# youngsm/chroma-lite

Hardware: AMD Instinct MI355X
Metric: propagated photons/sec, 29k-PMT detector, 10M isotropic photons, 1/2/4/8 GPUs (higher is better)
Workload: dtype f32

## Files before the change

chroma-lite_amd/chroma/gpu/_native.py:

```python
import ctypes
import os

_LIBDIR = os.path.join(os.path.dirname(os.path.dirname(os.path.abspath(__file__))), '_lib')
DEVICE_PROFILE = os.environ.get('CHROMA_DEVICE_PROFILE', '').strip().lower() in ('1', 'true', 'yes', 'on')
_LIBPATH = os.path.join(_LIBDIR, 'libchroma_amd_prof.so' if DEVICE_PROFILE else 'libchroma_amd.so')
_LIBPATH = os.environ.get('CHROMA_AMD_LIB', _LIBPATH)

c_u32 = ctypes.c_uint32
c_i32 = ctypes.c_int32
c_u64 = ctypes.c_uint64
c_f32 = ctypes.c_float
c_vp = ctypes.c_void_p
P_f32 = ctypes.POINTER(ctypes.c_float)
P_u32 = ctypes.POINTER(ctypes.c_uint32)


class MaterialDesc(ctypes.Structure):
    _fields_ = [('num_comp', c_u32), ('refractive_index', c_vp), ('absorption_length', c_vp),
                ('scattering_length', c_vp), ('comp_reemission_prob', c_vp),
                ('comp_reemission_wvl_cdf', c_vp), ('comp_reemission_time_cdf', c_vp),
                ('comp_absorption_length', c_vp)]


class SurfaceDesc(ctypes.Structure):
# ... 46 lines not shown
                ('tail_long_ticks', c_u64), ('tail_long_walk_ticks', c_u64), ('tail_long_walk_iterations', c_u64),
                ('host_syncs', c_u32), ('tail_long_paired_steps', c_u32), ('trace_launch_rays', c_u32 * 32)]


class KernelAttr(ctypes.Structure):
    _fields_ = [('private_bytes', c_u64), ('lds_bytes', c_u64), ('vgprs', ctypes.c_int32),
                ('max_threads', ctypes.c_int32), ('name', ctypes.c_char * 96)]


_SIGNATURES = {
    'chr_geometry_create': (c_i32, [ctypes.POINTER(GeometryDesc), ctypes.POINTER(c_vp)]),
    'chr_geometry_destroy': (c_i32, [c_vp]),
    'chr_geometry_device_bytes': (c_i32, [c_vp, ctypes.POINTER(c_u64)]),
    'chr_walk_lone_timing': (c_i32, [c_vp, c_vp, c_u32, c_u32, c_u32, c_i32, c_vp, c_vp]),
    'chr_geometry_phys_words': (c_i32, [c_vp, ctypes.POINTER(ctypes.c_uint32), ctypes.POINTER(ctypes.c_uint32)]),
    'chr_init_rng': (c_i32, [c_vp, c_u32, c_u64, c_u64, c_vp]),
    'chr_rng_download': (c_i32, [c_vp, c_u32, c_vp, c_vp]),
    'chr_propagate_scratch_words': (c_u64, [c_u32]),
    'chr_propagate_chunk': (c_i32, [c_vp, ctypes.POINTER(PhotonsDesc), c_vp, c_u32, c_i32, c_i32, c_vp, c_vp,
                                    c_i32, c_i32, c_i32, c_vp, c_vp]),
    'chr_propagate': (c_i32, [c_vp, ctypes.POINTER(PhotonsDesc), c_u32, c_u32, c_u32, c_vp, c_u32, c_i32, c_i32,
                              c_i32, c_i32, c_i32, ctypes.POINTER(PropagateStats), c_vp]),
    'chr_propagate_batches': (c_i32, [c_vp, ctypes.POINTER(PhotonsDesc), c_vp, c_vp, c_vp, c_u32, c_vp, c_u32, c_i32,
                                      c_i32, c_i32, c_i32, c_i32, ctypes.POINTER(PropagateStats), c_vp]),
    'chr_photon_hits': (c_i32, [ctypes.POINTER(PhotonsDesc), c_i32, c_i32, c_u32, c_vp, c_vp,
                                ctypes.POINTER(PhotonsDesc), c_vp, ctypes.POINTER(c_u32), c_vp]),
    'chr_select_photons': (c_i32, [ctypes.POINTER(PhotonsDesc), c_i32, c_i32, c_u32, ctypes.POINTER(PhotonsDesc),
                                   ctypes.POINTER(c_u32), c_vp]),
    'chr_copy_photon_queue': (c_i32, [ctypes.POINTER(PhotonsDesc), c_i32, c_i32, c_vp, ctypes.POINTER(PhotonsDesc),
                                      c_vp]),
# ... 92 lines not shown
    if rc != 0:
        msg = lib().chr_last_error().decode(errors='replace')
        raise NativeError('%s failed (status %d): %s' % (what, rc, msg))
    return rc


call_hook = None


def call(name, *args):
    if call_hook is not None:
        return call_hook(name, lambda: check(getattr(lib(), name)(*args), name))
    return check(getattr(lib(), name)(*args), name)


def kernel_info():
    out = []
    for which in range(4):
        a = KernelAttr()
        call('chr_kernel_info', which, ctypes.byref(a))
        out.append(dict(name=a.name.decode(), private_bytes=int(a.private_bytes), lds_bytes=int(a.lds_bytes),
                        vgprs=int(a.vgprs), max_threads=int(a.max_threads)))
    return out


def set_host_threads(n):
    call('chr_set_host_threads', int(n))


def host_threads():
    return int(lib().chr_get_host_threads())
```

chroma-lite_amd/chroma/gpu/geometry.py:

```python
import ctypes
import time

import numpy as np

from chroma.gpu import _native, wide_bvh
from chroma.gpu import gpuarray as ga
from chroma.gpu.packing import PackedGeometry
from chroma.gpu.tools import format_size
from chroma.log import logger


class GPUGeometry(object):
    def __init__(self, geometry, wavelengths=None, times=None, print_usage=False, min_free_gpu_mem=300e6):
        t0 = time.time()
        if getattr(geometry, 'bvh', None) is None:
            from chroma.loader import load_bvh
            geometry.bvh = load_bvh(geometry)
        self.packed = PackedGeometry(geometry, wavelengths=wavelengths, times=times)
        t1 = time.time()
        wide, source = wide_bvh.obtain(geometry.bvh, self.packed)
        t2 = time.time()
        handle = ctypes.c_void_p()
        try:
            _native.call('chr_geometry_create_wide', ctypes.byref(self.packed.desc()), ctypes.byref(wide.desc()),
# ... 44 lines not shown
        if getattr(self, '_triangles', None) is None:
            from chroma.gpu.tools import to_uint3
            self._triangles = ga.to_gpu(to_uint3(self.packed.triangles))
        return self._triangles

    def device_bytes(self):
        b = ctypes.c_uint64()
        _native.call('chr_geometry_device_bytes', self._handle, ctypes.byref(b))
        return b.value

    def phys_words(self):
        hot, total = ctypes.c_uint32(), ctypes.c_uint32()
        _native.call('chr_geometry_phys_words', self._handle, ctypes.byref(hot), ctypes.byref(total))
        return hot.value, total.value

    def device_usage_str(self):
        return 'device usage: geometry %s (%d triangles, %d BVH nodes)' % (
            format_size(self.device_bytes()), len(self.packed.triangles), len(self.packed.nodes))

    def print_device_usage(self):
        print(self.device_usage_str())

    def __del__(self):
        h = getattr(self, '_handle', None)
        if h is not None and h.value:
            try:
                _native.lib().chr_geometry_destroy(h)
            except Exception:
                pass
            self._handle = ctypes.c_void_p()
# ... 1 lines not shown
```

chroma-lite_amd/csrc/device_geometry.h:

```cpp
#pragma once
#include <vector>

#include <cstdint>

#include "../../include/chroma_amd.h"

namespace chr {

constexpr uint32_t TIME_INDEX_BUCKETS = 4096;

struct DevMaterial {
    uint32_t num_comp;
    uint32_t refractive_index, absorption_length, scattering_length;
    uint32_t comp_reemission_prob, comp_reemission_wvl_cdf, comp_absorption_length;
    uint32_t comp_reemission_time_cdf;
    uint32_t comp_time_index;
};

struct DevSurface {
    uint32_t present, model, transmissive;
    float thickness;
    uint32_t detect, absorb, reemit, reflect_diffuse, reflect_specular, eta, k, reemission_cdf;
    uint32_t dichroic_nangles, dichroic_angles, dichroic_reflect, dichroic_transmit;
    uint32_t angular_nangles, angular_angles, angular_transmit, angular_reflect_specular,
// ... 11 lines not shown
    const uint4 *wnodes;
    const float4 *wtri;
    uint32_t nwnodes, nwtri;
    uint32_t wstride;
    float ox, oy, oz, scale;
    float wbound;
    uint32_t nnodes, ntriangles, nwireplanes;
    uint32_t wl_n;
    float wl_start, wl_step;
    uint32_t t_n;
    float t_start, t_step;
    const uint32_t *phys;
    uint32_t phys_words, mat_off, surf_off;
    uint32_t phys_hot_words;
    const float *tables_g;
};

}

struct chr_geometry {
    chr::DevGeom dev;
    void *d_dev;
    int device;
    uint64_t bytes;
    void *allocs[16];
    int nallocs;
    std::vector<uint4> *h_ref_nodes;
    bool ref_tri_pending;
};
namespace chr {
// ... 5 lines not shown
```

chroma-lite_amd/csrc/geometry.cpp:

```cpp
#include <hip/hip_runtime_api.h>

#include <algorithm>
#include <cmath>
#include <cstdlib>
#include <cstring>
#include <mutex>
#include <new>
#include <string>
#include <unordered_map>
#include <vector>

#include "../../include/chroma_amd.h"
#include "common.h"
#include "slab_plane.h"
#include "wide_bvh.h"
#include "device_geometry.h"

namespace chr {
std::string &last_error() {
    static thread_local std::string msg;
    return msg;
}
}

// ... 100 lines not shown
    const int rc = run();
    if (prev != g->device) (void)hipSetDevice(prev);
    return rc;
}

extern "C" int chr_geometry_device_bytes(const chr_geometry *g, uint64_t *bytes) {
    if (!g || !bytes) return chr::fail(CHR_ERR_INVALID, "chr_geometry_device_bytes: null argument");
    *bytes = g->bytes;
    return CHR_OK;
}

extern "C" int chr_geometry_phys_words(const chr_geometry *g, uint32_t *hot_words, uint32_t *total_words) {
    if (!g || !hot_words || !total_words) return chr::fail(CHR_ERR_INVALID, "chr_geometry_phys_words: null argument");
    *hot_words = g->dev.phys_hot_words;
    *total_words = g->dev.phys_words;
    return CHR_OK;
}

struct Stager {
    static constexpr size_t CHUNK = 64u << 20;
    hipStream_t stream = nullptr;
    void *buf[2] = {nullptr, nullptr};
    hipEvent_t ev[2] = {nullptr, nullptr};
    bool used[2] = {false, false};
    std::vector<uint8_t> pageable;
    int init() {
        if (hipStreamCreateWithFlags(&stream, hipStreamNonBlocking) != hipSuccess) stream = nullptr;
        for (int k = 0; k < 2 && stream; ++k) {
            if (hipHostMalloc(&buf[k], CHUNK, hipHostMallocDefault) != hipSuccess ||
                hipEventCreateWithFlags(&ev[k], hipEventDisableTiming) != hipSuccess) {
// ... 175 lines not shown

        if ((rc = dev_upload(g, d->h_material_codes, (size_t)d->ntriangles * 4, &p))) throw rc;
        dg.material_codes = (const uint32_t *)p;

        Blob blob, comp;
        const uint32_t W1 = d->wavelength_n + 1, T1 = d->time_n + 1;
        std::vector<chr::DevMaterial> mats(d->nmaterials);
        for (uint32_t i = 0; i < d->nmaterials; ++i) {
            const chr_material_desc &m = d->materials[i];
            chr::DevMaterial &o = mats[i];
            if (!m.refractive_index || !m.absorption_length || !m.scattering_length) {
                rc = chr::fail(CHR_ERR_INVALID, "material %u: missing table", i);
                throw rc;
            }
            o.num_comp = m.num_comp;
            o.refractive_index = blob.add(m.refractive_index, W1);
            o.absorption_length = blob.add(m.absorption_length, W1);
            o.scattering_length = blob.add(m.scattering_length, W1);
            const size_t nc = m.num_comp;
            o.comp_reemission_prob = blob.add(m.comp_reemission_prob, nc * W1);
            o.comp_reemission_wvl_cdf = blob.add(m.comp_reemission_wvl_cdf, nc * W1);
            o.comp_absorption_length = blob.add(m.comp_absorption_length, nc * W1);
            o.comp_reemission_time_cdf = comp.add(m.comp_reemission_time_cdf, nc * T1);
            o.comp_time_index = ~0u;
            std::vector<uint32_t> idx;
            if (nc && chr::time_cdf_index(m.comp_reemission_time_cdf, m.num_comp, d->time_n, T1, idx))
                o.comp_time_index = comp.add(idx.data(), idx.size());
        }
        std::vector<chr::DevSurface> surfs(d->nsurfaces > 0 ? d->nsurfaces : 1);
        std::memset(surfs.data(), 0, surfs.size() * sizeof(chr::DevSurface));
        for (uint32_t i = 0; i < d->nsurfaces; ++i) {
            const chr_surface_desc &s = d->surfaces[i];
            chr::DevSurface &o = surfs[i];
            o.present = s.present ? 1u : 0u;
            if (!s.present) continue;
            o.model = s.model; o.transmissive = s.transmissive; o.thickness = s.thickness;
            o.detect = blob.add(s.detect, W1);
            o.absorb = blob.add(s.absorb, W1);
            o.reemit = blob.add(s.reemit, W1);
            o.reflect_diffuse = blob.add(s.reflect_diffuse, W1);
            o.reflect_specular = blob.add(s.reflect_specular, W1);
            o.eta = blob.add(s.eta, W1);
            o.k = blob.add(s.k, W1);
            o.reemission_cdf = blob.add(s.reemission_cdf, W1);
            if (s.model == CHR_SURFACE_DICHROIC && s.dichroic_nangles == 0) {
                rc = chr::fail(CHR_ERR_INVALID, "surface %u: dichroic model without DichroicProps", i);
                throw rc;
            }
            if (s.model == CHR_SURFACE_ANGULAR && s.angular_nangles == 0) {
                rc = chr::fail(CHR_ERR_INVALID, "surface %u: angular model without AngularProps", i);
                throw rc;
// ... 32 lines not shown
            phys.resize(phys.size() + comp.data.size());
            std::memcpy(phys.data() + hot, comp.data.data(), comp.data.size() * 4);
            phys.resize((phys.size() + 3) & ~(size_t)3, 0u);
            if ((rc = dev_upload(g, phys.data(), phys.size() * 4, &p))) throw rc;
            dg.phys = (const uint32_t *)p;
            dg.phys_words = (uint32_t)phys.size();
            dg.phys_hot_words = hot;
            dg.mat_off = mat_off;
            dg.surf_off = surf_off;
            dg.tables = (const float *)p;
            dg.tables_g = (const float *)p;
            dg.materials = (const chr::DevMaterial *)(dg.phys + mat_off);
            dg.surfaces = (const chr::DevSurface *)(dg.phys + surf_off);
        }
        if (d->nwireplanes) {
            if ((rc = dev_upload(g, d->wireplanes, (size_t)d->nwireplanes * sizeof(chr_wireplane_desc), &p))) throw rc;
            dg.wireplanes = (const chr_wireplane_desc *)p;
        }
        if ((rc = dev_upload(g, &dg, sizeof(dg), &p))) throw rc;
        g->d_dev = p;
    } catch (int code) {
        chr_geometry_destroy(g);
        return code;
    } catch (const std::bad_alloc &) {
        chr_geometry_destroy(g);
        return chr::fail(CHR_ERR_NOMEM, "chr_geometry_create: host allocation failed");
    }
    *out = g;
    return CHR_OK;
}
// ... 10 lines not shown
```

chroma-lite_amd/csrc/propagate.hip:

```cpp
#include <hip/hip_runtime.h>
#include <rocprim/device/device_radix_sort.hpp>

#include <algorithm>
#include <cstdint>
#include <cstdio>
#include <cstdlib>
#include <cstring>
#include <functional>
#include <type_traits>
#include <vector>

#include "../../include/chroma_amd.h"
#include "../../include/chroma_fmath.h"
#include "../../include/chroma_rng.h"
#include "common.h"
#include "device_geometry.h"
#include "device_math.h"
#include "sampling.h"
#include "slab_plane.h"
#include "wide_bvh.h"

namespace chr {

constexpr int BLOCK = 256;
constexpr int STACK_SIZE = 1000;
constexpr int STACK_LDS = 24;
constexpr uint32_t DEAD_MASK = CHR_NO_HIT | CHR_BULK_ABSORB | CHR_SURFACE_DETECT | CHR_SURFACE_ABSORB | CHR_NAN_ABORT;
constexpr float WEIGHT_LOWER_THRESHOLD = 0.0001f;
constexpr float SPEED_OF_LIGHT = 299.792458f;
constexpr float T_NEG_EPS = -9.99999997e-07f;
constexpr float T_ONE_EPS = 1.00000095367431640625f;
constexpr float T_POS_EPS = 9.99999997e-07f;

enum { BREAK = 0, CONTINUE = 1, PASS = 2 };

struct Photon {
    V3 pos, dir, pol;
    float wavelength, time, weight;
    uint32_t history;
// ... 792 lines not shown
            const double len = sqrt(vn_hit * vn_hit + nn_hit * nn_hit);
            if (len <= 0.0) continue;
            const V3 nl = v3((float)((vn_hit / len) * vx + (nn_hit / len) * nx),
                             (float)((vn_hit / len) * vy + (nn_hit / len) * ny),
                             (float)((vn_hit / len) * vz + (nn_hit / len) * nz));
            a_distance = (float)t;
            a_surface = wp.surface_index;
            a_inner = wp.material_inner_index;
            a_outer = wp.material_outer_index;
            a_normal_raw = nl;
            a_dot_raw = dot(nl, -p.dir);
        }
    }
}

template <bool REC, bool WIRES = true>
__device__ __forceinline__ void finish_fill(const DevGeom &g, State &s, Photon &p, int mesh_triangle) {
    int m1, m2;
    bool use_analytic = false;
    int a_surface = -1, a_inner = -1, a_outer = -1;
    V3 a_normal_raw = v3(0.0f, 0.0f, 0.0f);
    float a_dot_raw = 0.0f, a_distance = 1e30f;
    if (WIRES && g.nwireplanes > 0) {
        const float best_distance = (mesh_triangle == -1) ? 1e30f : s.distance;
        wireplanes(g, p, best_distance, a_surface, a_inner, a_outer, a_normal_raw, a_dot_raw, a_distance);
        if (a_surface >= 0) use_analytic = ((double)a_distance + 1e-12 < (double)best_distance);
    }
    if (use_analytic) {
        s.distance = a_distance;
        s.surface_index = a_surface;
        p.last_hit = -2;
        if (a_dot_raw > 0.0f) { m1 = a_outer; m2 = a_inner; s.normal = a_normal_raw; s.inside_to_outside = false; }
        else { m1 = a_inner; m2 = a_outer; s.normal = -a_normal_raw; s.inside_to_outside = true; }
    } else if (mesh_triangle != -1) {
        V3 e1, e3;
        int tid;
        uint32_t code;
        if constexpr (REC) {
// ... 66 lines not shown
    float cos_theta = 2.0f * chr_cosf((chr_acosf(__builtin_fmaf(-2.0f, u, 1.0f)) - 2 * PI_F) / 3.0f);
    if (cos_theta > 1.0f) cos_theta = 1.0f;
    else if (cos_theta < -1.0f) cos_theta = -1.0f;
    const float theta = chr_acosf(cos_theta);
    const float phi = chr_uniform(&rng, 0.0f, 2.0f * PI_F);
    p.dir = pick_new_direction(p.pol, theta, phi);
    if (1.0f - chr_fabsf(cos_theta) < 1e-6f)
        p.pol = pick_new_direction(p.pol, PI_F / 2.0f, phi);
    else
        p.pol = v3(__builtin_fmaf(-cos_theta, p.dir.x, p.pol.x), __builtin_fmaf(-cos_theta, p.dir.y, p.pol.y),
                   __builtin_fmaf(-cos_theta, p.dir.z, p.pol.z));
    p.dir = p.dir / norm(p.dir);
    p.pol = p.pol / norm(p.pol);
}

__device__ __forceinline__ int propagate_to_boundary(const DevGeom &g, Photon &p, State &s, chr_xorwow &rng, int use_weights,
                                     int scatter_first) {
    float absorption_distance = -s.absorption_length * chr_logf(chr_uniform01(&rng));
    float scattering_distance = -s.scattering_length * chr_logf(chr_uniform01(&rng));
    if (use_weights && p.weight > WEIGHT_LOWER_THRESHOLD) absorption_distance = 1e30f;
    else use_weights = 0;
    if (scatter_first == 1) {
        const float scatter_prob = 1.0f - chr_expf(-s.distance / s.scattering_length);
        if (scatter_prob > WEIGHT_LOWER_THRESHOLD) {
            int i = 0;
            while (i < 1000 && scattering_distance > s.distance) {
                scattering_distance = -s.scattering_length * chr_logf(chr_uniform01(&rng));
                i++;
            }
            p.weight *= scatter_prob;
// ... 1 lines not shown
    } else if (scatter_first == -1) {
        const float no_scatter_prob = chr_expf(-s.distance / s.scattering_length);
        if (no_scatter_prob > WEIGHT_LOWER_THRESHOLD) {
            int i = 0;
            while (i < 1000 && scattering_distance <= s.distance) {
                scattering_distance = -s.scattering_length * chr_logf(chr_uniform01(&rng));
                i++;
            }
            p.weight *= no_scatter_prob;
        }
    }
    if (absorption_distance <= scattering_distance) {
        if (absorption_distance <= s.distance) {
            p.time = p.time + absorption_distance / (SPEED_OF_LIGHT / s.n1);
            p.pos = axpy(absorption_distance, p.dir, p.pos);
            const DevMaterial &m = g.materials[s.material1];
            if (m.num_comp == 0) {
                p.last_hit = -1;
                p.history |= CHR_BULK_ABSORB;
                return BREAK;
            }
            const uint32_t W1 = g.wl_n + 1, T1 = g.t_n + 1;
            const float usc = chr_uniform01(&rng);
            float prob = 0.0f;
            uint32_t comp;
            for (comp = 0;; comp++) {
                const float comp_abs = interp_property(g, p.wavelength, g.tables + m.comp_absorption_length + comp * W1);
                prob += s.absorption_length / comp_abs;
                if (usc < prob || comp + 1 == m.num_comp) break;
            }
// ... 34 lines not shown
    }
    if (use_weights) p.weight *= chr_expf(-s.distance / s.absorption_length);
    p.pos = axpy(s.distance, p.dir, p.pos);
    p.time = p.time + s.distance / (SPEED_OF_LIGHT / s.n1);
    return PASS;
}

__device__ __forceinline__ void propagate_at_boundary(Photon &p, const State &s, chr_xorwow &rng) {
    const float incident_angle = get_theta(s.normal, -p.dir);
    const float refracted_angle = chr_asinf((chr_sinf(incident_angle) * s.n1) / s.n2);
    V3 ipn = cross(p.dir, s.normal);
    const float ipn_len = norm(ipn);
    if (ipn_len < 1e-6f) ipn = p.pol; else ipn = ipn / ipn_len;
    const float nc = dot(p.pol, ipn);
    const float normal_probability = nc * nc;
    float rc;
    if (chr_uniform01(&rng) < normal_probability) {
        rc = -chr_sinf(incident_angle - refracted_angle) / chr_sinf(incident_angle + refracted_angle);
        if ((chr_uniform01(&rng) < rc * rc) || chr_isnan(refracted_angle)) {
            p.dir = rotate(s.normal, incident_angle, ipn);
            p.history |= CHR_REFLECT_SPECULAR;
        } else {
            p.dir = rotate(s.normal, PI_F - refracted_angle, ipn);
        }
        p.pol = ipn;
    } else {
        rc = chr_tanf(incident_angle - refracted_angle) / chr_tanf(incident_angle + refracted_angle);
        if ((chr_uniform01(&rng) < rc * rc) || chr_isnan(refracted_angle)) {
            p.dir = rotate(s.normal, incident_angle, ipn);
            p.history |= CHR_REFLECT_SPECULAR;
        } else {
            p.dir = rotate(s.normal, PI_F - refracted_angle, ipn);
        }
        p.pol = cross(ipn, p.dir);
        p.pol = p.pol / norm(p.pol);
    }
}

__device__ __forceinline__ int specular_reflector(Photon &p, const State &s) {
    const float incident_angle = get_theta(s.normal, -p.dir);
    V3 ipn = cross(p.dir, s.normal);
    ipn = ipn / norm(ipn);
    p.dir = rotate(s.normal, incident_angle, ipn);
    p.history |= CHR_REFLECT_SPECULAR;
    return CONTINUE;
}

__device__ __forceinline__ int diffuse_reflector(Photon &p, const State &s, chr_xorwow &rng) {
    float ndotv;
    do {
        p.dir = uniform_sphere(rng);
// ... 212 lines not shown
    float rd = __builtin_fmaf(t, rdf[ihi] - rdf[iidx], rdf[iidx]);
    float ap = 1.0f - tp - rs - rd;
    if (use_weights && p.weight > WEIGHT_LOWER_THRESHOLD && ap < (1.0f - WEIGHT_LOWER_THRESHOLD)) {
        const float survive = 1.0f - ap;
        ap = 0.0f;
        p.weight *= survive;
        tp /= survive; rs /= survive; rd /= survive;
    }
    const float us = chr_uniform01(&rng);
    if (us < ap) { p.history |= CHR_SURFACE_ABSORB; return BREAK; }
    if (us < ap + tp) { p.history |= CHR_SURFACE_TRANSMIT; return PASS; }
    if (us < ap + tp + rs) return specular_reflector(p, s);
    return diffuse_reflector(p, s, rng);
}

__device__ __forceinline__ int propagate_at_surface(const DevGeom &g, Photon &p, const State &s, chr_xorwow &rng,
                                                    int use_weights) {
    const DevSurface &sf = g.surfaces[s.surface_index];
    if (sf.model == CHR_SURFACE_COMPLEX) return propagate_complex(g, p, s, rng, sf, use_weights);
    if (sf.model == CHR_SURFACE_WLS) return propagate_at_wls(g, p, s, rng, sf, use_weights);
    if (sf.model == CHR_SURFACE_DICHROIC) return propagate_at_dichroic(g, p, s, rng, sf);
    if (sf.model == CHR_SURFACE_ANGULAR) return propagate_at_angular(g, p, s, rng, sf, use_weights);
    const float *T = g.tables;
    float detect = interp_property(g, p.wavelength, T + sf.detect);
    float absorb = interp_property(g, p.wavelength, T + sf.absorb);
    float reflect_diffuse = interp_property(g, p.wavelength, T + sf.reflect_diffuse);
    float reflect_specular = interp_property(g, p.wavelength, T + sf.reflect_specular);
    const float us = chr_uniform01(&rng);
    if (use_weights && p.weight > WEIGHT_LOWER_THRESHOLD && absorb < (1.0f - WEIGHT_LOWER_THRESHOLD)) {
        const float survive = 1.0f - absorb;
        absorb = 0.0f;
        p.weight *= survive;
        detect /= survive; reflect_diffuse /= survive; reflect_specular /= survive;
    }
    if (use_weights && detect > 0.0f) {
        p.history |= CHR_SURFACE_DETECT;
        p.weight *= detect;
// ... 229 lines not shown
};
template <bool KNOWN = false>
__device__ __forceinline__ void fetch_queued(const PropagateArgs &a, uint32_t q, QueuedPhoton &f,
                                             uint32_t pid = 0xFFFFFFFFu) {
    f.pid = (KNOWN || pid != 0xFFFFFFFFu) ? pid : a.input_queue[q];
    f.history = a.flags[f.pid] & 0xFFFFu;
    f.pos = load3(a.pos, f.pid);
    f.dir = load3(a.dir, f.pid);
    f.pol = load3(a.pol, f.pid);
    f.wavelength = a.wl[f.pid];
    f.time = a.t[f.pid];
    f.weight = a.weights[f.pid];
    f.last_hit = a.last_hit[f.pid];
    f.hit = a.hits[q];
}
template <int MINW, bool WIRES = true>
__global__ __launch_bounds__(BLOCK, MINW) void shade_kernel(const DevGeom *__restrict__ gdev, PropagateArgs a,
                                                            uint32_t cap) {
    if (a.mode && *a.mode != a.want) return;
    CHR_PHYS_LDS(phys_lds, SHADE_PHYS_WORDS);
    const DevGeom g = phys_cache(*gdev, phys_lds, SHADE_PHYS_WORDS);
    const uint32_t slot = blockIdx.x * BLOCK + threadIdx.x;
    const uint32_t n = a.dev_n ? *a.dev_n - 1u : (uint32_t)a.nthreads;
    if (slot >= cap || (slot & ~63u) >= n) return;
    chr_xorwow rng;
    bool have_rng = false;
    enum { P_FILL, P_PHYS, P_OTHER };
    Prof<3> pf;
    pf.start(P_OTHER);
    auto clampq = [n](uint32_t q) { return q < n ? q : n - 1u; };
    QueuedPhoton nx;
// ... 16 lines not shown
            p.wavelength = cur.wavelength;
            p.time = cur.time;
            p.last_hit = cur.last_hit;
            p.weight = cur.weight;
            const float prod = ((((p.dir.x * p.dir.y) * p.dir.z) * p.pos.x) * p.pos.y) * p.pos.z;
            if (chr_isnan(prod)) {
                p.history |= CHR_NO_HIT | CHR_NAN_ABORT;
            } else {
                State s;
                const int tri = cur.hit.x;
                s.distance = __int_as_float(cur.hit.y);
                pf.tick(P_FILL);
                pf.call(P_FILL);
                Watch wt;
                wt.begin(1u, cur.pid, a.pos, pos, slot, p.pos, p.dir, p.last_hit);
                finish_fill<true, WIRES>(g, s, p, tri);
                wt.filled(tri, s);
                pf.tick(P_PHYS);
                if (p.last_hit != -1) {
                    pf.call(P_PHYS);
                    int command = propagate_to_boundary(g, p, s, rng, a.use_weights, a.scatter_first);
                    if (command == PASS && s.surface_index != -1)
                        command = propagate_at_surface(g, p, s, rng, a.use_weights);
                    if (command == PASS) propagate_at_boundary(p, s, rng);
                }
                wt.end(p.pos, p.history, p.time);
                pf.tick(P_OTHER);
            }
            alive = (p.history & DEAD_MASK) == 0;
        }
        asm volatile("" ::"v"(nx.pid), "v"(nx.history), "v"(nx.pos.x), "v"(nx.pos.y), "v"(nx.pos.z), "v"(nx.dir.x),
                     "v"(nx.dir.y), "v"(nx.dir.z), "v"(nx.pol.x), "v"(nx.pol.y), "v"(nx.pol.z));
        asm volatile("" ::"v"(nx.wavelength), "v"(nx.time), "v"(nx.weight), "v"(nx.last_hit), "v"(nx.hit.x),
                     "v"(nx.hit.y), "v"(pid2));
        if (valid) {
            const uint32_t pid = cur.pid;
            store3(a.pos, pid, p.pos);
            store3(a.dir, pid, p.dir);
            store3(a.pol, pid, p.pol);
            a.wl[pid] = p.wavelength;
            a.t[pid] = p.time;
            a.flags[pid] = p.history;
            a.last_hit[pid] = p.last_hit;
            a.weights[pid] = p.weight;
        }
        const unsigned long long mask = __ballot(alive);
        if ((slot & 63u) == 0) a.alive_masks[qb >> 6] = mask;
    };
    uint32_t qb = slot & ~63u;
    if (qb < n) {
        body(qb);
        qb += cap;
        pos += cap;
    }
    for (; qb < n; qb += cap, pos += cap) body(qb);
    if (have_rng) store_rng(a, slot, rng);
#ifdef CHR_DEVICE_PROFILE
    pf.tick(P_OTHER);
    prof_add(CHR_PROF_FILL_MATERIAL, pf.calls[P_FILL], pf.cyc[P_FILL]);
    prof_add(CHR_PROF_SHADE_PHYSICS, pf.calls[P_PHYS], pf.cyc[P_PHYS]);
    prof_add(CHR_PROF_SHADE_OTHER, 0ull, pf.cyc[P_OTHER]);
    prof_add(CHR_PROF_SHADE_KERNEL, 1ull, pf.total());
#endif
}


constexpr int TAIL_STACK = 128;
constexpr int TAIL_TRI = 4 * 64;

__device__ __forceinline__ unsigned long long dpp_min8(unsigned long long k) {
// ... 863 lines not shown
    __device__ __forceinline__ void mark(int i) {
        const unsigned long long now = __builtin_amdgcn_s_memtime();
        if (on) cyc[i] += now - t;
        t = now;
    }
    __device__ __forceinline__ void flush() {
        prof_add(CHR_PROF_LONG_WALK, steps, cyc[LP_WALK]);
        prof_add(CHR_PROF_LONG_FILL, 0ull, cyc[LP_FILL]);
        prof_add(CHR_PROF_LONG_TO_BOUNDARY, 0ull, cyc[LP_TO_BOUNDARY]);
        prof_add(CHR_PROF_LONG_AT_BOUNDARY, 0ull, cyc[LP_AT_BOUNDARY]);
        prof_add(CHR_PROF_LONG_OTHER, 0ull, cyc[LP_OTHER]);
    }
};
#endif

template <int MINW, bool WIRES = true>
__global__ __launch_bounds__(BLOCK, MINW) void propagate_tail_kernel(const DevGeom *__restrict__ gdev, PropagateArgs a,
                                                                     uint32_t cap) {
    __shared__ uint32_t stacks[(BLOCK / 8) * TAIL_STACK * 2];
    __shared__ uint32_t tris[(BLOCK / 64) * 2 * TAIL_TRI];
    const uint32_t tid = blockIdx.x * BLOCK + threadIdx.x;
    const uint32_t lane = __lane_id();
    if (a.mode && *a.mode != a.want) return;
    if (a.prio) __builtin_amdgcn_s_setprio(3);
    __shared__ uint32_t box_s[PB_WORDS];
    CHR_LDS uint32_t *box = (CHR_LDS uint32_t *)box_s;
    if (threadIdx.x == 0) {
        box_s[PB_STATE] = PS_IDLE;
        box_s[PB_IDLE] = 0u;
        box_s[PB_WORKERS] = BLOCK / 64;
        box_s[PB_ABORT] = 0u;
// ... 205 lines not shown
            }
            pf.tick(P_OTHER);
        }
        if (walk) {
            pf.tick(P_PHYS);
            if (sub == 0) {
                pf.call(P_WALK);
                pf.call(P_PHYS);
                const V3 inv = v3(1.0f / p.dir.x, 1.0f / p.dir.y, 1.0f / p.dir.z);
                if (!(chr_isfinite(inv.x) && chr_isfinite(inv.y) && chr_isfinite(inv.z))) flat++;
            }
            lpf.mark(LP_WALK);
            s.distance = dist;
            Watch wt;
            wt.begin(2u, sub == 0 ? pid : 0xFFFFFFFFu, a.pos, q, slot, p.pos, p.dir, p.last_hit);
            finish_fill<true, WIRES>(g, s, p, tri);
            wt.filled(tri, s);
            up_chain = up_node != 0xFFFFFFFFu
                           ? gld(reinterpret_cast<const uint32_t *>(g.wnodes + (size_t)g.wstride * (up_node & WIDE_NODE_MASK)) +
                                 24 + sub)
                           : 0xFFFFFFFFu;
            lpf.mark(LP_FILL);
            bool stop = p.last_hit == -1;
            if (!stop) {
                int command = propagate_to_boundary(g, p, s, rng, a.use_weights, scatter_first);
                lpf.mark(LP_TO_BOUNDARY);
                scatter_first = 0;
                if (command == BREAK) {
                    stop = true;
                } else if (command == PASS) {
                    if (s.surface_index != -1) {
                        command = propagate_at_surface(g, p, s, rng, a.use_weights);
                        if (command == BREAK) stop = true;
                    }
                    if (command == PASS) propagate_at_boundary(p, s, rng);
                }
                lpf.mark(LP_AT_BOUNDARY);
            }
            wt.end(p.pos, p.history, p.time);
            pf.tick(P_OTHER);
            if (stop) finish();
        }
    }
    if (!wq && have_rng && sub == 0) store_rng(a, slot, rng);
    if (sub == 0 && overflow) atomicAdd(a.counters, overflow);
    if (sub == 0 && flat && a.diag) atomicAdd(a.diag, flat);
    serve();
// ... 828 lines not shown

typedef void (*propagate_step_fn)(const DevGeom *, PropagateArgs, uint32_t);
typedef void (*trace_fn)(const DevGeom *, TraceArgs);
struct StepVariant {
    propagate_step_fn fn;
    trace_fn trace = nullptr;
    trace_fn trace_gather = nullptr;
    propagate_step_fn shade = nullptr;
    int trace_waves = 4;
    int trace_block = BLOCK;
    propagate_step_fn tail = nullptr;
    int tail_group = 0;
    int binned = 0;
};
static constexpr uint32_t kBinFirstMin = 1u << 20;
static StepVariant select_step_variant(const chr_geometry *g) {
    const char *e = getenv("CHR_PROPAGATE_VARIANT");
    int v = e ? atoi(e) : 0;
    const bool wires = g->dev.nwireplanes > 0;
    StepVariant sv;
    if (g->dev.nwnodes == 0 || v == kExactVariant) {
        sv.fn = propagate_step_kernel<8, 4, 0>;
        return sv;
    }
    if (!wide_queue_ok(g) || v == 4 || v == 6) {
        sv.fn = (v == 3 || v == 5 || v == 6) ? propagate_step_kernel<8, 4, kWalkSched, true>
                                              : propagate_step_kernel<8, 4, kWalkSched>;
        return sv;
    }
    switch (v) {
        case 2: sv.fn = propagate_step_kernel<8, 4, kWalk>; break;
        case 3: sv.fn = propagate_step_kernel<8, 4, kWalk, true>; break;
        case 5:
            sv.fn = propagate_step_kernel<8, 4, kWalk, true>;
            sv.trace = trace_kernel<true, 6, 12, 4, 32>;
            sv.trace_gather = trace_kernel<true, 6, 12, 4, 32, true>;
            sv.shade = wires ? shade_kernel<3> : shade_kernel<3, false>;
            sv.tail = wires ? propagate_tail_kernel<kTailWaves> : propagate_tail_kernel<kTailWaves, false>;
            sv.tail_group = 8;
            sv.binned = 2;
            break;
        default:
            sv.fn = propagate_step_kernel<8, 4, kWalk>;
            sv.trace = trace_kernel<false, 6, 12, 4, 48>;
            sv.trace_gather = trace_kernel<false, 6, 12, 4, 48, true>;
            sv.shade = wires ? shade_kernel<3> : shade_kernel<3, false>;
            sv.tail = wires ? propagate_tail_kernel<kTailWaves> : propagate_tail_kernel<kTailWaves, false>;
            sv.tail_group = 8;
            sv.binned = v == 7 ? 1 : (v == 8 ? 0 : 2);
            break;
    }
    static const bool lds_caps = []() {
        const int sb = (int)(SHADE_PHYS_WORDS * 4), tb = (int)(TAIL_PHYS_WORDS * 4);
        (void)hipFuncSetAttribute((const void *)shade_kernel<3>, hipFuncAttributeMaxDynamicSharedMemorySize, sb);
        (void)hipFuncSetAttribute((const void *)shade_kernel<3, false>, hipFuncAttributeMaxDynamicSharedMemorySize, sb);
        (void)hipFuncSetAttribute((const void *)propagate_tail_kernel<kTailWaves>,
                                  hipFuncAttributeMaxDynamicSharedMemorySize, tb);
        (void)hipFuncSetAttribute((const void *)propagate_tail_kernel<kTailWaves, false>,
                                  hipFuncAttributeMaxDynamicSharedMemorySize, tb);
        (void)hipGetLastError();
        return true;
    }();
    (void)lds_caps;
    return sv;
}

static bool pair_walk_enabled();
static uint32_t walk_up_mode();
static int launch_chunk(const chr_geometry *g, const chr_photons *ph, uint32_t *rng, uint32_t nslots, int32_t first,
                        int32_t nthreads, const uint32_t *in_queue, uint32_t *out_queue, int32_t max_steps,
                        int32_t use_weights, int32_t scatter_first, uint32_t *scratch, hipStream_t stream,
                        hipEvent_t ev0 = nullptr, hipEvent_t ev1 = nullptr) {
    const uint32_t nwords = (uint32_t)((nthreads + 63) / 64);
    uint32_t *counters = scratch;
// ... 1000 lines not shown
                                    int32_t stride, void *stream) {
    if (!photons_ok(ph)) return chr::fail(CHR_ERR_INVALID, "duplicate: null argument");
    if (nphotons <= 0 || copies <= 0) return CHR_OK;
    hipLaunchKernelGGL(duplicate_kernel, dim3(grid_for(nphotons)), dim3(BLOCK), 0, (hipStream_t)stream, to_ptrs(ph),
                       first_photon, nphotons, copies, stride);
    CHR_HIP_CHECK(hipGetLastError());
    return CHR_OK;
}

extern "C" int chr_kernel_info(int32_t which, chr_kernel_attr *out) {
    if (!out) return chr::fail(CHR_ERR_INVALID, "chr_kernel_info: null output");
    const void *fn = nullptr;
    const char *name = nullptr;
    switch (which) {
        case 0: fn = (const void *)trace_kernel<false, 6, 12, 4, 48>; name = "chr::trace_kernel<false,6,12,4,48>"; break;
        case 1: fn = (const void *)shade_kernel<3>; name = "chr::shade_kernel<3>"; break;
        case 2: fn = (const void *)propagate_tail_kernel<kTailWaves>; name = "chr::propagate_tail_kernel<2>"; break;
        case 3: fn = (const void *)propagate_step_kernel<8, 4, kWalk>; name = "chr::propagate_step_kernel<8,4,2006>"; break;
        default: return chr::fail(CHR_ERR_INVALID, "chr_kernel_info: unknown kernel %d", which);
    }
    hipFuncAttributes fa;
    CHR_HIP_CHECK(hipFuncGetAttributes(&fa, fn));
    out->private_bytes = fa.localSizeBytes;
    out->lds_bytes = fa.sharedSizeBytes;
    out->vgprs = fa.numRegs;
    out->max_threads = fa.maxThreadsPerBlock;
    std::snprintf(out->name, sizeof(out->name), "%s", name);
    return CHR_OK;
}

extern "C" int chr_distance_to_mesh(const chr_geometry *g, uint32_t n, const float *d_origin, const float *d_direction,
                                    float *d_distance, void *stream) {
    if (!g || !d_origin || !d_direction || !d_distance) return chr::fail(CHR_ERR_INVALID, "distance_to_mesh: null argument");
// ... 236 lines not shown
```

include/chroma_amd.h:

```cpp
#ifndef CHROMA_AMD_H
#define CHROMA_AMD_H

#include <stdint.h>
#include <stddef.h>

#ifdef __cplusplus
extern "C" {
#endif

enum chr_status {
    CHR_OK = 0,
    CHR_ERR_INVALID = 1,
    CHR_ERR_HIP = 2,
    CHR_ERR_NOMEM = 3,
    CHR_ERR_STACK = 4
};

enum chr_history {
    CHR_NO_HIT = 1u << 0, CHR_BULK_ABSORB = 1u << 1, CHR_SURFACE_DETECT = 1u << 2,
    CHR_SURFACE_ABSORB = 1u << 3, CHR_RAYLEIGH_SCATTER = 1u << 4, CHR_REFLECT_DIFFUSE = 1u << 5,
    CHR_REFLECT_SPECULAR = 1u << 6, CHR_SURFACE_REEMIT = 1u << 7, CHR_SURFACE_TRANSMIT = 1u << 8,
    CHR_BULK_REEMIT = 1u << 9, CHR_CHERENKOV = 1u << 10, CHR_SCINTILLATION = 1u << 11,
    CHR_NAN_ABORT = 1u << 15
};
// ... 45 lines not shown
    float world_origin[3];
    float world_scale;
    uint32_t wavelength_n; float wavelength_start, wavelength_step;
    uint32_t time_n; float time_start, time_step;
    const chr_material_desc *materials;
    const chr_surface_desc *surfaces;
    const chr_wireplane_desc *wireplanes;
} chr_geometry_desc;

typedef struct chr_geometry chr_geometry;

int chr_geometry_create(const chr_geometry_desc *desc, chr_geometry **out);
int chr_geometry_destroy(chr_geometry *g);
int chr_geometry_device_bytes(const chr_geometry *g, uint64_t *bytes);
int chr_geometry_phys_words(const chr_geometry *g, uint32_t *hot_words, uint32_t *total_words);

typedef struct chr_photons {
    float *d_pos, *d_dir, *d_pol;
    float *d_wavelengths, *d_t, *d_weights;
    uint32_t *d_flags;
    int32_t *d_last_hit_triangles;
    uint32_t *d_evidx;
} chr_photons;

int chr_init_rng(uint32_t *d_states, uint32_t nslots, uint64_t seed, uint64_t offset, void *stream);
int chr_init_rng_subseq(uint32_t *d_states, uint32_t nslots, uint64_t seed, uint64_t first_subsequence,
                        uint64_t offset, void *stream);
int chr_rng_download(const uint32_t *d_states, uint32_t nslots, uint32_t *h_out, void *stream);

uint64_t chr_propagate_scratch_words(uint32_t nthreads);
// ... 257 lines not shown
```

Baseline: 536.0 million.

## Specialize shade and tail kernels on geometry physics features, branchless Fresnel

The geometry upload now records which physics features are present: wireplanes, complex, WLS, dichroic or angular surfaces, and reemitting materials. The host picks a shade and tail kernel instantiation (plain, no-wires or full) so unused surface models and reemission paths are compiled out, which cuts register pressure and branch divergence. Specular Fresnel reflection is also rewritten to use sincos with selects instead of divergent branches. The do-while loop with asm register pins is meant to steer the compiler's scheduling. Risks are more kernel variants to compile and maintain, and slightly different float results in the Fresnel path.

```diff
diff --git a/chroma-lite_amd/chroma/gpu/_native.py b/chroma-lite_amd/chroma/gpu/_native.py
--- a/chroma-lite_amd/chroma/gpu/_native.py
+++ b/chroma-lite_amd/chroma/gpu/_native.py
@@ -84,6 +84,7 @@
     'chr_geometry_device_bytes': (c_i32, [c_vp, ctypes.POINTER(c_u64)]),
     'chr_walk_lone_timing': (c_i32, [c_vp, c_vp, c_u32, c_u32, c_u32, c_i32, c_vp, c_vp]),
     'chr_geometry_phys_words': (c_i32, [c_vp, ctypes.POINTER(ctypes.c_uint32), ctypes.POINTER(ctypes.c_uint32)]),
+    'chr_geometry_phys_features': (c_i32, [c_vp, ctypes.POINTER(ctypes.c_uint32)]),
     'chr_init_rng': (c_i32, [c_vp, c_u32, c_u64, c_u64, c_vp]),
     'chr_rng_download': (c_i32, [c_vp, c_u32, c_vp, c_vp]),
     'chr_propagate_scratch_words': (c_u64, [c_u32]),
@@ -206,9 +207,14 @@
     return check(getattr(lib(), name)(*args), name)
 
 
+PHYS_FEATURES = {'wires': 1 << 0, 'complex': 1 << 1, 'wls': 1 << 2, 'dichroic': 1 << 3, 'angular': 1 << 4,
+                 'reemission': 1 << 5}
+KERNEL_INFO_COUNT = 8
+
+
 def kernel_info():
     out = []
-    for which in range(4):
+    for which in range(KERNEL_INFO_COUNT):
         a = KernelAttr()
         call('chr_kernel_info', which, ctypes.byref(a))
         out.append(dict(name=a.name.decode(), private_bytes=int(a.private_bytes), lds_bytes=int(a.lds_bytes),
diff --git a/chroma-lite_amd/chroma/gpu/geometry.py b/chroma-lite_amd/chroma/gpu/geometry.py
--- a/chroma-lite_amd/chroma/gpu/geometry.py
+++ b/chroma-lite_amd/chroma/gpu/geometry.py
@@ -82,6 +82,11 @@
         _native.call('chr_geometry_phys_words', self._handle, ctypes.byref(hot), ctypes.byref(total))
         return hot.value, total.value
 
+    def phys_features(self):
+        out = ctypes.c_uint32()
+        _native.call('chr_geometry_phys_features', self._handle, ctypes.byref(out))
+        return out.value
+
     def device_usage_str(self):
         return 'device usage: geometry %s (%d triangles, %d BVH nodes)' % (
             format_size(self.device_bytes()), len(self.packed.triangles), len(self.packed.nodes))
diff --git a/chroma-lite_amd/csrc/device_geometry.h b/chroma-lite_amd/csrc/device_geometry.h
--- a/chroma-lite_amd/csrc/device_geometry.h
+++ b/chroma-lite_amd/csrc/device_geometry.h
@@ -49,6 +49,7 @@
     uint32_t phys_words, mat_off, surf_off;
     uint32_t phys_hot_words;
     const float *tables_g;
+    uint32_t phys_features;
 };
 
 }
diff --git a/chroma-lite_amd/csrc/geometry.cpp b/chroma-lite_amd/csrc/geometry.cpp
--- a/chroma-lite_amd/csrc/geometry.cpp
+++ b/chroma-lite_amd/csrc/geometry.cpp
@@ -138,6 +138,12 @@
     if (!g || !hot_words || !total_words) return chr::fail(CHR_ERR_INVALID, "chr_geometry_phys_words: null argument");
     *hot_words = g->dev.phys_hot_words;
     *total_words = g->dev.phys_words;
+    return CHR_OK;
+}
+
+extern "C" int chr_geometry_phys_features(const chr_geometry *g, uint32_t *out) {
+    if (!g || !out) return chr::fail(CHR_ERR_INVALID, "chr_geometry_phys_features: null argument");
+    *out = g->dev.phys_features;
     return CHR_OK;
 }
 
@@ -343,6 +349,7 @@
                 throw rc;
             }
             o.num_comp = m.num_comp;
+            if (m.num_comp) dg.phys_features |= CHR_PHYS_REEMISSION;
             o.refractive_index = blob.add(m.refractive_index, W1);
             o.absorption_length = blob.add(m.absorption_length, W1);
             o.scattering_length = blob.add(m.scattering_length, W1);
@@ -364,6 +371,8 @@
             o.present = s.present ? 1u : 0u;
             if (!s.present) continue;
             o.model = s.model; o.transmissive = s.transmissive; o.thickness = s.thickness;
+            if (s.model >= CHR_SURFACE_COMPLEX && s.model <= CHR_SURFACE_ANGULAR)
+                dg.phys_features |= CHR_PHYS_COMPLEX << (s.model - CHR_SURFACE_COMPLEX);
             o.detect = blob.add(s.detect, W1);
             o.absorb = blob.add(s.absorb, W1);
             o.reemit = blob.add(s.reemit, W1);
@@ -426,6 +435,7 @@
             dg.surfaces = (const chr::DevSurface *)(dg.phys + surf_off);
         }
         if (d->nwireplanes) {
+            dg.phys_features |= CHR_PHYS_WIRES;
             if ((rc = dev_upload(g, d->wireplanes, (size_t)d->nwireplanes * sizeof(chr_wireplane_desc), &p))) throw rc;
             dg.wireplanes = (const chr_wireplane_desc *)p;
         }
diff --git a/chroma-lite_amd/csrc/propagate.hip b/chroma-lite_amd/csrc/propagate.hip
--- a/chroma-lite_amd/csrc/propagate.hip
+++ b/chroma-lite_amd/csrc/propagate.hip
@@ -23,6 +23,9 @@
 namespace chr {
 
 constexpr int BLOCK = 256;
+constexpr uint32_t PHYS_PLAIN = 0u;
+constexpr uint32_t PHYS_FULL = CHR_PHYS_ALL;
+constexpr uint32_t PHYS_NOWIRES = PHYS_FULL & ~(uint32_t)CHR_PHYS_WIRES;
 constexpr int STACK_SIZE = 1000;
 constexpr int STACK_LDS = 24;
 constexpr uint32_t DEAD_MASK = CHR_NO_HIT | CHR_BULK_ABSORB | CHR_SURFACE_DETECT | CHR_SURFACE_ABSORB | CHR_NAN_ABORT;
@@ -845,14 +848,14 @@
     }
 }
 
-template <bool REC, bool WIRES = true>
+template <bool REC, uint32_t FEAT = PHYS_FULL>
 __device__ __forceinline__ void finish_fill(const DevGeom &g, State &s, Photon &p, int mesh_triangle) {
     int m1, m2;
     bool use_analytic = false;
     int a_surface = -1, a_inner = -1, a_outer = -1;
     V3 a_normal_raw = v3(0.0f, 0.0f, 0.0f);
     float a_dot_raw = 0.0f, a_distance = 1e30f;
-    if (WIRES && g.nwireplanes > 0) {
+    if constexpr ((FEAT & CHR_PHYS_WIRES) != 0) if (g.nwireplanes > 0) {
         const float best_distance = (mesh_triangle == -1) ? 1e30f : s.distance;
         wireplanes(g, p, best_distance, a_surface, a_inner, a_outer, a_normal_raw, a_dot_raw, a_distance);
         if (a_surface >= 0) use_analytic = ((double)a_distance + 1e-12 < (double)best_distance);
@@ -949,6 +952,7 @@
     p.pol = p.pol / norm(p.pol);
 }
 
+template <uint32_t FEAT = PHYS_FULL>
 __device__ __forceinline__ int propagate_to_boundary(const DevGeom &g, Photon &p, State &s, chr_xorwow &rng, int use_weights,
                                      int scatter_first) {
     float absorption_distance = -s.absorption_length * chr_logf(chr_uniform01(&rng));
@@ -980,6 +984,11 @@
         if (absorption_distance <= s.distance) {
             p.time = p.time + absorption_distance / (SPEED_OF_LIGHT / s.n1);
             p.pos = axpy(absorption_distance, p.dir, p.pos);
+            if constexpr (!(FEAT & CHR_PHYS_REEMISSION)) {
+                p.last_hit = -1;
+                p.history |= CHR_BULK_ABSORB;
+                return BREAK;
+            }
             const DevMaterial &m = g.materials[s.material1];
             if (m.num_comp == 0) {
                 p.last_hit = -1;
@@ -1044,6 +1053,7 @@
     if (ipn_len < 1e-6f) ipn = p.pol; else ipn = ipn / ipn_len;
     const float nc = dot(p.pol, ipn);
     const float normal_probability = nc * nc;
+#ifdef CHR_FRESNEL_BRANCHY
     float rc;
     if (chr_uniform01(&rng) < normal_probability) {
         rc = -chr_sinf(incident_angle - refracted_angle) / chr_sinf(incident_angle + refracted_angle);
@@ -1065,6 +1075,22 @@
         p.pol = cross(ipn, p.dir);
         p.pol = p.pol / norm(p.pol);
     }
+#else
+    float sd, cd, ss, cs;
+    chr_sincosf(incident_angle - refracted_angle, &sd, &cd);
+    chr_sincosf(incident_angle + refracted_angle, &ss, &cs);
+    const bool s_pol = chr_uniform01(&rng) < normal_probability;
+    const float rc = s_pol ? -sd / ss : (sd / cd) / (ss / cs);
+    const bool reflect = (chr_uniform01(&rng) < rc * rc) || chr_isnan(refracted_angle);
+    p.dir = rotate(s.normal, reflect ? incident_angle : PI_F - refracted_angle, ipn);
+    if (reflect) p.history |= CHR_REFLECT_SPECULAR;
+    if (s_pol) {
+        p.pol = ipn;
+    } else {
+        p.pol = cross(ipn, p.dir);
+        p.pol = p.pol / norm(p.pol);
+    }
+#endif
 }
 
 __device__ __forceinline__ int specular_reflector(Photon &p, const State &s) {
@@ -1307,13 +1333,18 @@
     return diffuse_reflector(p, s, rng);
 }
 
+template <uint32_t FEAT = PHYS_FULL>
 __device__ __forceinline__ int propagate_at_surface(const DevGeom &g, Photon &p, const State &s, chr_xorwow &rng,
                                                     int use_weights) {
     const DevSurface &sf = g.surfaces[s.surface_index];
-    if (sf.model == CHR_SURFACE_COMPLEX) return propagate_complex(g, p, s, rng, sf, use_weights);
-    if (sf.model == CHR_SURFACE_WLS) return propagate_at_wls(g, p, s, rng, sf, use_weights);
-    if (sf.model == CHR_SURFACE_DICHROIC) return propagate_at_dichroic(g, p, s, rng, sf);
-    if (sf.model == CHR_SURFACE_ANGULAR) return propagate_at_angular(g, p, s, rng, sf, use_weights);
+    if constexpr ((FEAT & CHR_PHYS_COMPLEX) != 0)
+        if (sf.model == CHR_SURFACE_COMPLEX) return propagate_complex(g, p, s, rng, sf, use_weights);
+    if constexpr ((FEAT & CHR_PHYS_WLS) != 0)
+        if (sf.model == CHR_SURFACE_WLS) return propagate_at_wls(g, p, s, rng, sf, use_weights);
+    if constexpr ((FEAT & CHR_PHYS_DICHROIC) != 0)
+        if (sf.model == CHR_SURFACE_DICHROIC) return propagate_at_dichroic(g, p, s, rng, sf);
+    if constexpr ((FEAT & CHR_PHYS_ANGULAR) != 0)
+        if (sf.model == CHR_SURFACE_ANGULAR) return propagate_at_angular(g, p, s, rng, sf, use_weights);
     const float *T = g.tables;
     float detect = interp_property(g, p.wavelength, T + sf.detect);
     float absorb = interp_property(g, p.wavelength, T + sf.absorb);
@@ -1573,7 +1604,7 @@
     f.last_hit = a.last_hit[f.pid];
     f.hit = a.hits[q];
 }
-template <int MINW, bool WIRES = true>
+template <int MINW, uint32_t FEAT = PHYS_FULL>
 __global__ __launch_bounds__(BLOCK, MINW) void shade_kernel(const DevGeom *__restrict__ gdev, PropagateArgs a,
                                                             uint32_t cap) {
     if (a.mode && *a.mode != a.want) return;
@@ -1620,14 +1651,14 @@
                 pf.call(P_FILL);
                 Watch wt;
                 wt.begin(1u, cur.pid, a.pos, pos, slot, p.pos, p.dir, p.last_hit);
-                finish_fill<true, WIRES>(g, s, p, tri);
+                finish_fill<true, FEAT>(g, s, p, tri);
                 wt.filled(tri, s);
                 pf.tick(P_PHYS);
                 if (p.last_hit != -1) {
                     pf.call(P_PHYS);
-                    int command = propagate_to_boundary(g, p, s, rng, a.use_weights, a.scatter_first);
+                    int command = propagate_to_boundary<FEAT>(g, p, s, rng, a.use_weights, a.scatter_first);
                     if (command == PASS && s.surface_index != -1)
-                        command = propagate_at_surface(g, p, s, rng, a.use_weights);
+                        command = propagate_at_surface<FEAT>(g, p, s, rng, a.use_weights);
                     if (command == PASS) propagate_at_boundary(p, s, rng);
                 }
                 wt.end(p.pos, p.history, p.time);
@@ -1654,12 +1685,22 @@
         if ((slot & 63u) == 0) a.alive_masks[qb >> 6] = mask;
     };
     uint32_t qb = slot & ~63u;
-    if (qb < n) {
+#ifdef CHR_SHADE_PEEL
+    body(qb);
+    qb += cap;
+    pos += cap;
+    for (; qb < n; qb += cap, pos += cap) body(qb);
+#else
+    asm volatile("" ::"v"(nx.pid), "v"(nx.history), "v"(nx.pos.x), "v"(nx.pos.y), "v"(nx.pos.z), "v"(nx.dir.x),
+                 "v"(nx.dir.y), "v"(nx.dir.z), "v"(nx.pol.x), "v"(nx.pol.y), "v"(nx.pol.z));
+    asm volatile("" ::"v"(nx.wavelength), "v"(nx.time), "v"(nx.weight), "v"(nx.last_hit), "v"(nx.hit.x),
+                 "v"(nx.hit.y), "v"(pid2));
+    do {
         body(qb);
         qb += cap;
         pos += cap;
-    }
-    for (; qb < n; qb += cap, pos += cap) body(qb);
+    } while (qb < n);
+#endif
     if (have_rng) store_rng(a, slot, rng);
 #ifdef CHR_DEVICE_PROFILE
     pf.tick(P_OTHER);
@@ -2553,7 +2594,7 @@
 };
 #endif
 
-template <int MINW, bool WIRES = true>
+template <int MINW, uint32_t FEAT = PHYS_FULL>
 __global__ __launch_bounds__(BLOCK, MINW) void propagate_tail_kernel(const DevGeom *__restrict__ gdev, PropagateArgs a,
                                                                      uint32_t cap) {
     __shared__ uint32_t stacks[(BLOCK / 8) * TAIL_STACK * 2];
@@ -2789,7 +2830,7 @@
             s.distance = dist;
             Watch wt;
             wt.begin(2u, sub == 0 ? pid : 0xFFFFFFFFu, a.pos, q, slot, p.pos, p.dir, p.last_hit);
-            finish_fill<true, WIRES>(g, s, p, tri);
+            finish_fill<true, FEAT>(g, s, p, tri);
             wt.filled(tri, s);
             up_chain = up_node != 0xFFFFFFFFu
                            ? gld(reinterpret_cast<const uint32_t *>(g.wnodes + (size_t)g.wstride * (up_node & WIDE_NODE_MASK)) +
@@ -2798,14 +2839,14 @@
             lpf.mark(LP_FILL);
             bool stop = p.last_hit == -1;
             if (!stop) {
-                int command = propagate_to_boundary(g, p, s, rng, a.use_weights, scatter_first);
+                int command = propagate_to_boundary<FEAT>(g, p, s, rng, a.use_weights, scatter_first);
                 lpf.mark(LP_TO_BOUNDARY);
                 scatter_first = 0;
                 if (command == BREAK) {
                     stop = true;
                 } else if (command == PASS) {
                     if (s.surface_index != -1) {
-                        command = propagate_at_surface(g, p, s, rng, a.use_weights);
+                        command = propagate_at_surface<FEAT>(g, p, s, rng, a.use_weights);
                         if (command == BREAK) stop = true;
                     }
                     if (command == PASS) propagate_at_boundary(p, s, rng);
@@ -3664,10 +3705,26 @@
     int binned = 0;
 };
 static constexpr uint32_t kBinFirstMin = 1u << 20;
+static uint32_t phys_variant(const chr_geometry *g) {
+    const char *e = getenv("CHR_PHYS_FULL");
+    if (e && e[0] == '1') return PHYS_FULL;
+    const uint32_t f = g->dev.phys_features;
+    return f == 0u ? PHYS_PLAIN : ((f & CHR_PHYS_WIRES) ? PHYS_FULL : PHYS_NOWIRES);
+}
+static constexpr int kShadeWaves = 3;
+static propagate_step_fn shade_for(uint32_t feat) {
+    if (feat == PHYS_PLAIN) return shade_kernel<kShadeWaves, PHYS_PLAIN>;
+    return feat == PHYS_NOWIRES ? shade_kernel<kShadeWaves, PHYS_NOWIRES> : shade_kernel<kShadeWaves, PHYS_FULL>;
+}
+static propagate_step_fn tail_for(uint32_t feat) {
+    if (feat == PHYS_PLAIN) return propagate_tail_kernel<kTailWaves, PHYS_PLAIN>;
+    return feat == PHYS_NOWIRES ? propagate_tail_kernel<kTailWaves, PHYS_NOWIRES>
+                                : propagate_tail_kernel<kTailWaves, PHYS_FULL>;
+}
 static StepVariant select_step_variant(const chr_geometry *g) {
     const char *e = getenv("CHR_PROPAGATE_VARIANT");
     int v = e ? atoi(e) : 0;
-    const bool wires = g->dev.nwireplanes > 0;
+    const uint32_t feat = phys_variant(g);
     StepVariant sv;
     if (g->dev.nwnodes == 0 || v == kExactVariant) {
         sv.fn = propagate_step_kernel<8, 4, 0>;
@@ -3685,8 +3742,8 @@
             sv.fn = propagate_step_kernel<8, 4, kWalk, true>;
             sv.trace = trace_kernel<true, 6, 12, 4, 32>;
             sv.trace_gather = trace_kernel<true, 6, 12, 4, 32, true>;
-            sv.shade = wires ? shade_kernel<3> : shade_kernel<3, false>;
-            sv.tail = wires ? propagate_tail_kernel<kTailWaves> : propagate_tail_kernel<kTailWaves, false>;
+            sv.shade = shade_for(feat);
+            sv.tail = tail_for(feat);
             sv.tail_group = 8;
             sv.binned = 2;
             break;
@@ -3694,20 +3751,18 @@
             sv.fn = propagate_step_kernel<8, 4, kWalk>;
             sv.trace = trace_kernel<false, 6, 12, 4, 48>;
             sv.trace_gather = trace_kernel<false, 6, 12, 4, 48, true>;
-            sv.shade = wires ? shade_kernel<3> : shade_kernel<3, false>;
-            sv.tail = wires ? propagate_tail_kernel<kTailWaves> : propagate_tail_kernel<kTailWaves, false>;
+            sv.shade = shade_for(feat);
+            sv.tail = tail_for(feat);
             sv.tail_group = 8;
             sv.binned = v == 7 ? 1 : (v == 8 ? 0 : 2);
             break;
     }
     static const bool lds_caps = []() {
         const int sb = (int)(SHADE_PHYS_WORDS * 4), tb = (int)(TAIL_PHYS_WORDS * 4);
-        (void)hipFuncSetAttribute((const void *)shade_kernel<3>, hipFuncAttributeMaxDynamicSharedMemorySize, sb);
-        (void)hipFuncSetAttribute((const void *)shade_kernel<3, false>, hipFuncAttributeMaxDynamicSharedMemorySize, sb);
-        (void)hipFuncSetAttribute((const void *)propagate_tail_kernel<kTailWaves>,
-                                  hipFuncAttributeMaxDynamicSharedMemorySize, tb);
-        (void)hipFuncSetAttribute((const void *)propagate_tail_kernel<kTailWaves, false>,
-                                  hipFuncAttributeMaxDynamicSharedMemorySize, tb);
+        for (uint32_t f : {PHYS_PLAIN, PHYS_NOWIRES, PHYS_FULL}) {
+            (void)hipFuncSetAttribute((const void *)shade_for(f), hipFuncAttributeMaxDynamicSharedMemorySize, sb);
+            (void)hipFuncSetAttribute((const void *)tail_for(f), hipFuncAttributeMaxDynamicSharedMemorySize, tb);
+        }
         (void)hipGetLastError();
         return true;
     }();
@@ -4738,9 +4793,13 @@
     const char *name = nullptr;
     switch (which) {
         case 0: fn = (const void *)trace_kernel<false, 6, 12, 4, 48>; name = "chr::trace_kernel<false,6,12,4,48>"; break;
-        case 1: fn = (const void *)shade_kernel<3>; name = "chr::shade_kernel<3>"; break;
-        case 2: fn = (const void *)propagate_tail_kernel<kTailWaves>; name = "chr::propagate_tail_kernel<2>"; break;
+        case 1: fn = (const void *)shade_for(PHYS_FULL); name = "chr::shade_kernel<3>"; break;
+        case 2: fn = (const void *)tail_for(PHYS_FULL); name = "chr::propagate_tail_kernel<2>"; break;
         case 3: fn = (const void *)propagate_step_kernel<8, 4, kWalk>; name = "chr::propagate_step_kernel<8,4,2006>"; break;
+        case 4: fn = (const void *)shade_for(PHYS_PLAIN); name = "chr::shade_kernel<3,PLAIN>"; break;
+        case 5: fn = (const void *)tail_for(PHYS_PLAIN); name = "chr::propagate_tail_kernel<2,PLAIN>"; break;
+        case 6: fn = (const void *)shade_for(PHYS_NOWIRES); name = "chr::shade_kernel<3,NOWIRES>"; break;
+        case 7: fn = (const void *)tail_for(PHYS_NOWIRES); name = "chr::propagate_tail_kernel<2,NOWIRES>"; break;
         default: return chr::fail(CHR_ERR_INVALID, "chr_kernel_info: unknown kernel %d", which);
     }
     hipFuncAttributes fa;
diff --git a/include/chroma_amd.h b/include/chroma_amd.h
--- a/include/chroma_amd.h
+++ b/include/chroma_amd.h
@@ -83,6 +83,12 @@
 int chr_geometry_destroy(chr_geometry *g);
 int chr_geometry_device_bytes(const chr_geometry *g, uint64_t *bytes);
 int chr_geometry_phys_words(const chr_geometry *g, uint32_t *hot_words, uint32_t *total_words);
+enum chr_phys_feature {
+    CHR_PHYS_WIRES = 1u << 0, CHR_PHYS_COMPLEX = 1u << 1, CHR_PHYS_WLS = 1u << 2,
+    CHR_PHYS_DICHROIC = 1u << 3, CHR_PHYS_ANGULAR = 1u << 4, CHR_PHYS_REEMISSION = 1u << 5,
+    CHR_PHYS_ALL = (1u << 6) - 1u
+};
+int chr_geometry_phys_features(const chr_geometry *g, uint32_t *out);
 
 typedef struct chr_photons {
     float *d_pos, *d_dir, *d_pol;
```

Result: no change. 539.4 million (median of 6 runs) (+0.6%).
